# aosokin/os2d

Measured on AMD Instinct MI355X. Metric: query-image-pairs/s (1280-px input, ResNet50, N-class), higher is better.
Workload: dtype fftx3 (as fft; the per-bin complex GEMM on the fp16 MFMA with spectra split into fp16 hi+lo, 3 MFMAs per product, fp32 accumulate)

## Files before the change

### os2d_amd/csrc/dft_mfma.h

```cpp
#pragma once

#ifndef DFT_DEV
#error "the includer defines DFT_DEV, DFT_TID, DFT_BID, DFT_GRID, DFT_LDS, DFT_BARRIER, DFT_MFMA, DFT_SHFL_XOR, DFT_SHFL_XOR_U32, DFT_BALLOT, DFT_FLAG, DFT_FLAG_SET, DFT_RAISE, DFT_UNIFORM"
#endif

#ifndef DFT_HD
#define DFT_HD static inline
#endif
#ifndef DFT_MEMBER
#define DFT_MEMBER inline
#endif
#ifndef DFT_LANDED
#define DFT_LANDED(X)
#endif
#ifndef DFT_SWAP1
#define DFT_SWAP1(V) DFT_SHFL_XOR(V, 1)
#endif
#ifndef DFT_FWD_PREFETCH_AFTER
#define DFT_FWD_PREFETCH_AFTER 2
#endif
#ifndef DFT_INV_PREFETCH_AFTER
#define DFT_INV_PREFETCH_AFTER 2
#endif
#ifndef DFT_PIPE_REGA
#define DFT_PIPE_REGA 1
#endif
#ifndef DFT_PIPE_LDS
#define DFT_PIPE_LDS 1
#endif
#ifndef DFT_SCHED_FENCE
#define DFT_SCHED_FENCE()
#endif
#ifndef DFT_STREAM_STORE
#define DFT_STREAM_STORE(P, V) (*(P) = (V))
#endif
#ifndef DFT_STAMP
#define DFT_STAMP(K)
#define DFT_STAMP_BEGIN()
#define DFT_STAMP_END(BASE)
#endif

#include "tile_common.h"

namespace os2d_dft {

typedef float f32x4u __attribute__((ext_vector_type(4), aligned(4)));

constexpr int DFT_THR = 512, DFT_WAVES = 8;
constexpr int DFT_G = 4;
constexpr int DFT_MAXP = 64;
constexpr int DFT_MAXV = 48;
constexpr int DFT_MAXWK = 96;
constexpr int DFT_KREG = 8;
constexpr int DFT_OUT_SHB = 0, DFT_OUT_SHB_BORDERS = 1, DFT_OUT_PLANES = 2;

struct DftPlan {
  int H, W;
  int P, Q, V, NBINS;
  int T, TY, TX, TH, TW;
  int oy, ox;
  int LH, LW;
  int RH;
  int Pp;
  int Wk;
  int N1;
  int M2;
  int Mx;
  int N2;
  int MA;
  int MB;
  int KB;
  int NBo;
  int G;
  int eT;
  int fast;
  unsigned inv_cg, inv_t, inv_tx, inv_c4, inv_v, inv_pq, inv_og, inv_kg, inv_pp;
  int lds_const, lds_union, lds_total;
};

DFT_HD int dft_round_up(int x, int m) { return (x + m - 1) / m * m; }
DFT_HD unsigned dft_magic(unsigned d) { return d > 1 ? (unsigned)(((1ull << 32) + d - 1) / d) : 0u; }

DFT_HD int dft_units_fqt(int P, int Q) { return (dft_round_up(Q, 16) / 8) * 2 * dft_round_up(Q + 2, 32); }
constexpr int DFT_R2_P = 64, DFT_R2_MATU = 8 * 2 * 64, DFT_R2_TWU = 16;
constexpr int DFT_R2_LDS_TW = 512;
DFT_HD bool dft_radix2(int P) { return P == DFT_R2_P; }
DFT_HD int dft_units_fp2(int P, int Q) {
  return dft_radix2(P) ? DFT_R2_MATU + DFT_R2_TWU : (2 * dft_round_up(P, 8) / 8) * 2 * dft_round_up(2 * P, 32);
}
DFT_HD int dft_units_e2(int P, int Q) { return (2 * dft_round_up(P, 8) / 8) * 2 * dft_round_up(2 * P, 32); }
DFT_HD int dft_units_gq(int P, int Q) { return (dft_round_up(Q + 2, 16) / 8) * 2 * dft_round_up(Q, 32); }
DFT_HD size_t dft_matrices_units(int P, int Q) {
  return (size_t)dft_units_fqt(P, Q) + dft_units_fp2(P, Q) + dft_units_e2(P, Q) + dft_units_gq(P, Q);
}

static inline bool dft_plan_transform(int LH, int LW, int RH, int ncols, int minP, int minQ, int G, DftPlan* pl) {
  pl->G = G;
  pl->P = dft_round_up(minP, 4);
  if (pl->P == 60) pl->P = DFT_R2_P;
  pl->Q = dft_round_up(minQ, 2);
  pl->V = pl->Q / 2 + 1;
  pl->NBINS = dft_round_up(pl->P * pl->V, 8);
  pl->LH = LH;
  pl->LW = LW;
  pl->RH = RH;
  pl->Pp = dft_round_up(pl->P, 8);
  pl->Wk = dft_round_up(LW, 16);
  pl->N1 = dft_round_up(2 * pl->V, 32);
  pl->M2 = dft_round_up(2 * pl->P, 32);
  pl->Mx = dft_round_up(G * pl->Pp, 32);
  pl->N2 = dft_round_up(G * pl->V, 32);
  pl->MA = dft_round_up(2 * RH, 32);
  pl->MB = G * (pl->MA / 2);
  pl->KB = dft_round_up(2 * pl->V, 16);
  pl->NBo = dft_round_up(ncols, 32);
  int e = 0;
  while ((1 << e) < pl->P) ++e;
  pl->eT = e + 1;
  if (pl->P > DFT_MAXP || pl->V > DFT_MAXV || pl->Wk > DFT_MAXWK || LH > pl->P || LW > pl->Q || RH > pl->P) return false;
  const int fqt = (pl->Wk / 8) * 2 * pl->N1 * 16, gq = (pl->KB / 8) * 2 * pl->NBo * 16;
  const int x = (pl->Wk / 8) * 2 * (pl->Mx + 1) * 16, r2 = (2 * pl->Pp / 8) * 2 * (pl->N2 + 1) * 16;
  const int xs = pl->V * (pl->P * 8 * G + 16);
  const int y2 = r2, tt = (pl->KB / 8) * 2 * (pl->MB + 1) * 16;
  int u = x;
  if (r2 > u) u = r2;
  if (xs > u) u = xs;
  if (y2 > u) u = y2;
  if (tt > u) u = tt;
  if (G == 8) {
    if (dft_radix2(pl->P)) return false;
    const int fp2 = (2 * pl->Pp / 8) * 2 * pl->M2 * 16;
    const int ca = fqt + fp2, cb = gq + fp2;
    pl->lds_const = ca > cb ? ca : cb;
    pl->lds_union = dft_round_up(u, 256);
    pl->lds_total = pl->lds_const + pl->lds_union + 1024;
    const int t1 = (pl->Mx / 32) * (pl->N1 / 32), t2 = (pl->M2 / 32) * (pl->N2 / 32), tA = (pl->MA / 32) * (pl->N2 / 32),
              tB = (pl->MB / 32) * (pl->NBo / 32);
    const int npos = pl->Pp * (pl->Wk / 4), nitem = G * pl->V * (pl->Pp / 8);
    return pl->lds_total <= 160 * 1024 && t1 <= 24 && t2 <= 24 && tA <= 24 && tB <= 24 && npos <= 2 * DFT_THR && nitem <= 3 * DFT_THR;
  }
  pl->lds_const = fqt > gq ? fqt : gq;
  pl->lds_union = dft_round_up(u, 256);
  pl->lds_total = pl->lds_const + pl->lds_union + 1024;
  return pl->lds_total <= 160 * 1024;
}

static inline void dft_set_tiles(DftPlan* pl, int H, int W, int TY, int TX, int TH, int TW) {
  pl->H = H;
  pl->W = W;
  pl->TY = TY;
  pl->TX = TX;
  pl->T = TY * TX;
  pl->TH = TH;
  pl->TW = TW;
  pl->oy = TY > 1 ? 3 : 0;
  pl->ox = TX > 1 ? 3 : 0;
  pl->fast = (pl->T == 1 && (W & 3) == 0) ? 1 : 0;
  pl->inv_t = dft_magic((unsigned)pl->T);
  pl->inv_tx = dft_magic((unsigned)TX);
  pl->inv_c4 = dft_magic((unsigned)(pl->Wk / 4));
  pl->inv_v = dft_magic((unsigned)pl->V);
  pl->inv_pq = dft_magic((unsigned)(pl->P / 4 * pl->G * 2));
  pl->inv_kg = dft_magic((unsigned)(pl->Pp / 8));
  pl->inv_pp = dft_magic((unsigned)pl->Pp);
}

struct DftSize {
  int P, Q;
};
static const DftSize DFT_CANONICAL[6] = {{36, 46}, {44, 54}, {48, 62}, {52, 68}, {56, 70}, {64, 84}};

static inline bool dft_make_plan_policy(int H, int W, int canonical, DftPlan* out, int G = DFT_G) {
  bool found = false;
  long best = 0;
  for (int TY = 1; TY <= 48; ++TY)
    for (int TX = 1; TX <= 48; ++TX) {
      const int TH = (H + TY - 1) / TY, TW = (W + TX - 1) / TX;
      if ((TY > 1 && (TY - 1) * TH >= H) || (TX > 1 && (TX - 1) * TW >= W)) continue;
      const int LH = TY > 1 ? TH + 6 : H, LW = TX > 1 ? TW + 6 : W;
      const int minP = TY > 1 ? TH + 6 : H + 3, minQ = TX > 1 ? TW + 6 : W + 3;
      if (minP > DFT_MAXP || minQ > 2 * (DFT_MAXV - 1)) continue;
      for (int k = 0; k < (canonical ? 6 : 1); ++k) {
        if (canonical && (DFT_CANONICAL[k].P < minP || DFT_CANONICAL[k].Q < minQ)) continue;
        DftPlan c = {};
        if (!dft_plan_transform(LH, LW, TY > 1 ? TH + 3 : H, TX > 1 ? TW + 3 : W, canonical ? DFT_CANONICAL[k].P : minP,
                                canonical ? DFT_CANONICAL[k].Q : minQ, G, &c))
          continue;
        dft_set_tiles(&c, H, W, TY, TX, TH, TW);
        const long cost = (long)c.T * c.NBINS;
        if (!found || cost < best) {
          found = true;
          best = cost;
          *out = c;
        }
      }
    }
  return found;
}

#ifndef OS2D_HOST_EMU
static inline int dft_size_policy() {
  static const int policy = [] {
    const char* e = getenv("OS2D_DFT_SIZES");
    return (e && (e[0] == 'e' || e[0] == '0')) ? 0 : 1;
  }();
  return policy;
}
#else
static inline int dft_size_policy() { return emu_dft_policy; }
#endif
static inline bool dft_make_plan(int H, int W, DftPlan* out) { return dft_make_plan_policy(H, W, dft_size_policy(), out); }
static inline bool dft_plan_g8(const DftPlan& base, DftPlan* out) {
  DftPlan c = {};
  if (!dft_plan_transform(base.LH, base.LW, base.RH, base.TX > 1 ? base.TW + 3 : base.W, base.P, base.Q, 8, &c)) return false;
  dft_set_tiles(&c, base.H, base.W, base.TY, base.TX, base.TH, base.TW);
  *out = c;
  return true;
}

constexpr int DFT_PBLK = 64;
DFT_HD size_t dft_spectra_pair0(int pr, int NBT, int NQ, int cstride, size_t* qstride) {
  const int pb = pr / DFT_PBLK, pl = pr - pb * DFT_PBLK;
  const int nbl = NBT - pb * DFT_PBLK < DFT_PBLK ? NBT - pb * DFT_PBLK : DFT_PBLK;
  *qstride = (size_t)nbl * cstride * 8;
  return ((size_t)pb * DFT_PBLK * NQ + pl) * cstride * 8;
}

DFT_DEV int dft_div(int x, unsigned magic) { return magic ? (int)(((unsigned long long)(unsigned)x * magic) >> 32) : x; }

DFT_DEV void dft_split4(float a, float b, float c, float d, u32x2* hi, u32x2* lo) {
  const f32x4 x = {a, b, c, d};
  const half4 h = __builtin_convertvector(x, half4);
  *hi = __builtin_bit_cast(u32x2, h);
#ifdef DFT_SPLIT_LO_PAIR
  u32x2 l;
  l[0] = DFT_SPLIT_LO_PAIR(a, b, (*hi)[0]);
  l[1] = DFT_SPLIT_LO_PAIR(c, d, (*hi)[1]);
  *lo = l;
#else
  const half4 l = __builtin_convertvector(x - __builtin_convertvector(h, f32x4), half4);
  *lo = __builtin_bit_cast(u32x2, l);
#endif
}

DFT_DEV half8 dft_frag(const u32x4* p) { return __builtin_bit_cast(half8, *p); }

DFT_DEV f32x16 dft_mma3(half8 ah, half8 al, half8 bh, half8 bl, f32x16 acc) {
  acc = DFT_MFMA(ah, bl, acc);
  acc = DFT_MFMA(al, bh, acc);
  acc = DFT_MFMA(ah, bh, acc);
  return acc;
}

template <int NT, int KS>
DFT_DEV void dft_product_rega(f32x16* acc, const half8* ah, const half8* al, int ksn, const u32x4* B, int bstride, int nt0,
                              int ntstep, int l31, int hw) {
  constexpr int KR = KS ? KS : DFT_KREG;
  half8 bh[2][NT], bl[2][NT];
#define DFT_REGA_READ(KSTEP, SET)                                                                                          \
  _Pragma("unroll") for (int j = 0; j < NT; ++j) {                                                                         \
    bh[SET][j] = dft_frag(B + (size_t)((2 * (KSTEP) + hw) * 2 + 0) * bstride + (nt0 + ntstep * j) * 32 + l31);             \
    bl[SET][j] = dft_frag(B + (size_t)((2 * (KSTEP) + hw) * 2 + 1) * bstride + (nt0 + ntstep * j) * 32 + l31);             \
  }
  if (DFT_PIPE_REGA) DFT_REGA_READ(0, 0)
#pragma unroll
  for (int ks = 0; ks < KR; ++ks) {
    if (KS || ks < ksn) {
      if (DFT_PIPE_REGA) {
        if (ks + 1 < KR && (KS || ks + 1 < ksn)) DFT_REGA_READ(ks + 1, (ks + 1) & 1)
        DFT_SCHED_FENCE();
      } else {
        DFT_REGA_READ(ks, ks & 1)
      }
#pragma unroll
      for (int j = 0; j < NT; ++j) acc[j] = dft_mma3(ah[ks], al[ks], bh[ks & 1][j], bl[ks & 1][j], acc[j]);
      if (DFT_PIPE_REGA) DFT_SCHED_FENCE();
    }
  }
#undef DFT_REGA_READ
}

template <int KS>
DFT_DEV void dft_product_rega_any(f32x16* acc, int ntiles, const half8* ah, const half8* al, int ksn, const u32x4* B, int bstride,
                                  int nt0, int ntstep, int l31, int hw) {
  if (ntiles == 3) dft_product_rega<3, KS>(acc, ah, al, ksn, B, bstride, nt0, ntstep, l31, hw);
  else if (ntiles == 2) dft_product_rega<2, KS>(acc, ah, al, ksn, B, bstride, nt0, ntstep, l31, hw);
  else if (ntiles == 1) dft_product_rega<1, KS>(acc, ah, al, ksn, B, bstride, nt0, ntstep, l31, hw);
}

template <int NT, bool SHARE, int NW, int PIPE_MODE>
DFT_DEV void dft_product_lds(f32x16* acc, int ks0, int ks1, const u32x4* A, int astride, const u32x4* B, int bstride, int t0, int mtn,
                             int l31, int hw) {
  constexpr int NA = SHARE ? 1 : NT;
  int tm[NT], tn[NT];
#pragma unroll
  for (int j = 0; j < NT; ++j) {
    const int t = t0 + NW * j;
    tn[j] = t / mtn;
    tm[j] = t - tn[j] * mtn;
  }
  half8 ah[2][NA], al[2][NA], bh[2][NT], bl[2][NT];
#define DFT_LDS_READ(KSTEP, SET)                                                                                           \
  {                                                                                                                        \
    const int kc_ = (KSTEP) < ks1 ? (KSTEP) : ks1 - 1;                                                                     \
    _Pragma("unroll") for (int j = 0; j < NA; ++j) {                                                                       \
      ah[SET][j] = dft_frag(A + (size_t)((2 * kc_ + hw) * 2 + 0) * astride + tm[j] * 32 + l31);                            \
      al[SET][j] = dft_frag(A + (size_t)((2 * kc_ + hw) * 2 + 1) * astride + tm[j] * 32 + l31);                            \
    }                                                                                                                      \
    _Pragma("unroll") for (int j = 0; j < NT; ++j) {                                                                       \
      bh[SET][j] = dft_frag(B + (size_t)((2 * kc_ + hw) * 2 + 0) * bstride + tn[j] * 32 + l31);                            \
      bl[SET][j] = dft_frag(B + (size_t)((2 * kc_ + hw) * 2 + 1) * bstride + tn[j] * 32 + l31);                            \
    }                                                                                                                      \
  }
#define DFT_LDS_MMA(SET)                                                                                                   \
  DFT_SCHED_FENCE();                                                                                                       \
  _Pragma("unroll") for (int j = 0; j < NT; ++j)                                                                           \
    acc[j] = dft_mma3(ah[SET][SHARE ? 0 : j], al[SET][SHARE ? 0 : j], bh[SET][j], bl[SET][j], acc[j]);                    \
  DFT_SCHED_FENCE();
  if (ks0 >= ks1) return;
  constexpr bool PIPE = PIPE_MODE == 2 || (PIPE_MODE == 1 && SHARE);
  if (!PIPE) {
    for (int ks = ks0; ks < ks1; ++ks) {
      DFT_LDS_READ(ks, 0)
      _Pragma("unroll") for (int j = 0; j < NT; ++j)
        acc[j] = dft_mma3(ah[0][SHARE ? 0 : j], al[0][SHARE ? 0 : j], bh[0][j], bl[0][j], acc[j]);
    }
    return;
  }
  DFT_LDS_READ(ks0, 0)
  int ks = ks0;
  for (; ks + 1 < ks1; ks += 2) {
    DFT_LDS_READ(ks + 1, 1)
    DFT_LDS_MMA(0)
    DFT_LDS_READ(ks + 2, 0)
    DFT_LDS_MMA(1)
  }
  if (ks < ks1) {
    DFT_LDS_MMA(0)
  }
#undef DFT_LDS_READ
#undef DFT_LDS_MMA
}

template <int NW, int PIPE_MODE>
DFT_DEV void dft_product_lds_any(f32x16* acc, int ntiles, int ks0, int ks1, const u32x4* A, int astride, const u32x4* B, int bstride,
                                 int t0, int mtn, int l31, int hw) {
  const bool share = mtn == NW;
  if (ntiles == 3) {
    if (share) dft_product_lds<3, true, NW, PIPE_MODE>(acc, ks0, ks1, A, astride, B, bstride, t0, mtn, l31, hw);
    else dft_product_lds<3, false, NW, PIPE_MODE>(acc, ks0, ks1, A, astride, B, bstride, t0, mtn, l31, hw);
  } else if (ntiles == 2) {
    if (share) dft_product_lds<2, true, NW, PIPE_MODE>(acc, ks0, ks1, A, astride, B, bstride, t0, mtn, l31, hw);
    else dft_product_lds<2, false, NW, PIPE_MODE>(acc, ks0, ks1, A, astride, B, bstride, t0, mtn, l31, hw);
  } else if (ntiles == 1) {
    dft_product_lds<1, true, NW, PIPE_MODE>(acc, ks0, ks1, A, astride, B, bstride, t0, mtn, l31, hw);
  }
}

DFT_DEV void dft_matrix_unit(int which, int unit, int P, int Q, const double* twP, const double* twQ, u32x4* out) {
  const int V = Q / 2 + 1;
  const bool r2 = which == 1 && dft_radix2(P);
  if (r2 && unit >= DFT_R2_MATU) {
    const int u = 2 * (unit - DFT_R2_MATU);
    u32x4 o;
    for (int t = 0; t < 4; ++t) o[t] = __builtin_bit_cast(unsigned, (float)twP[2 * u + t]);
    *out = o;
    return;
  }
  const int tws = r2 ? 2 : 1;
  if (r2) P /= 2;
  const int Pp = dft_round_up(P, 8);
  int cols, kidx, hl, col;
  double vals[8];
  if (which == 0) cols = dft_round_up(2 * V, 32);
  else if (which == 1 || which == 2) cols = dft_round_up(2 * P, 32);
  else cols = dft_round_up(Q, 32);
  col = unit % cols;
  hl = (unit / cols) & 1;
  kidx = unit / (2 * cols);
  for (int t = 0; t < 8; ++t) {
    const int k = kidx * 8 + t;
    double x = 0.0;
    if (which == 0) {
      const int v = col >> 1, ri = col & 1;
      if (k < Q && v < V) x = twQ[2 * (int)(((long long)v * k) % Q) + ri] * 16384.0;
    } else if (r2) {
      const int h = 8 * (2 * (kidx >> 1) + (t >> 2)) + 4 * (kidx & 1) + (t & 3), u = col & 31;
      if (kidx < 4) {
        const int a = (int)(((long long)u * h) % P) * tws;
// ... 283 lines not shown
      for (int j = 0; j < 3; ++j) {
        const int t = wv + NW * j;
        const int nt = ALDS ? t / mt2n : (wv >> 2) + (NW / 4) * j;
        const bool mine = ALDS ? t < mt2n * nt2n : (nt < nt2n && mt2 < mt2n);
        un[j] = mine ? nt : -1;
        um[j] = ALDS ? t - nt * mt2n : mt2;
        nt2w += mine ? 1 : 0;
#pragma unroll
        for (int r = 0; r < 16; ++r) xc[j][r] = 0.f;
      }
      const int itn = it + DFT_GRID < iters ? it + DFT_GRID : it;
      {
        if (ALDS) {
          dft_product_lds_any<NW, DFT_PIPE_LDS ? 2 : 0>(xc, nt2w, 0, ks2n, ldsP, pl.M2, ldsU, N2S, wv, mt2n, l31, hw);
          DFT_FWD_PREFETCH_SLOTS(itn, tl, 0, NSLOT)
        } else if (DFT_FWD_PREFETCH_AFTER == 1 || (DFT_FWD_PREFETCH_AFTER == 2 && KS2 > 0 && KS2 <= 6)) {
          dft_product_rega_any<KS2>(xc, nt2w, fp2h, fp2l, ks2n, ldsU, N2S, wv >> 2, NW / 4, l31, hw);
          DFT_FWD_PREFETCH_SLOTS(itn, tl, 0, NSLOT)
        } else {
          DFT_FWD_PREFETCH_SLOTS(itn, tl, 0, NSLOT)
          dft_product_rega_any<KS2>(xc, nt2w, fp2h, fp2l, ks2n, ldsU, N2S, wv >> 2, NW / 4, l31, hw);
        }
      }
      DFT_BARRIER();
      DFT_STAMP(3)

      const int XS = P * 8 * G + 16;
#pragma unroll
      for (int j = 0; j < 3; ++j) {
        if (un[j] < 0) continue;
        const int n2 = un[j] * 32 + l31;
        const int img = dft_div(n2, pl.inv_v), v = n2 - img * V;
#pragma unroll
        for (int q = 0; q < 4; ++q) {
          const int u0 = (um[j] * 32 + 8 * q + 4 * hw) >> 1;
          if (img < G && u0 < P) {
            const float sc = 1.0f / 4194304.0f;
            f32x4 o;
            o[0] = xc[j][4 * q] * sc;
            o[1] = xc[j][4 * q + 1] * sc;
            o[2] = xc[j][4 * q + 2] * sc;
            o[3] = xc[j][4 * q + 3] * sc;
            *reinterpret_cast<f32x4*>(ldsUb + (size_t)v * XS + (u0 >> 2) * (G * 32) + img * 32 + (u0 & 3) * 8) = o;
          }
        }
      }
      DFT_BARRIER();
      DFT_STAMP(4)
    }

    {
      const int XS = P * 8 * G + 16;
      const int per_v = (P / 4) * (G * 2), npieces = V * per_v;
      size_t qstride;
      float* dstbase = X + dft_spectra_pair0(pr_, NBT, pl.NBINS / 4, Cpad, &qstride) + (size_t)c0_ * 8;
      if (R2) {
        constexpr int per_h = (DFT_R2_P / 8) * (G * 2);
        for (int i = tl; i < V * per_h; i += THR) {
          const int v = i / per_h, rem = i - v * per_h;
          const int uq = rem / (2 * G), jj = rem - uq * (2 * G);
          const unsigned char* src = ldsUb + (size_t)v * XS + uq * (G * 32) + jj * 16;
          const f32x4 e = *reinterpret_cast<const f32x4*>(src);
          const f32x4 o = *reinterpret_cast<const f32x4*>(src + (DFT_R2_P / 8) * (G * 32));
          const f32x4 w = *reinterpret_cast<const f32x4*>(ldsTw + (4 * uq + 2 * (jj & 1)) * 8);
          f32x4 t;
          t[0] = w[0] * o[0] - w[1] * o[1];
          t[1] = w[0] * o[1] + w[1] * o[0];
          t[2] = w[2] * o[2] - w[3] * o[3];
          t[3] = w[2] * o[3] + w[3] * o[2];
          float* dst = dstbase + (size_t)(v * (P / 4) + uq) * qstride + jj * 4;
          DFT_STREAM_STORE(reinterpret_cast<f32x4*>(dst), e + t);
          DFT_STREAM_STORE(reinterpret_cast<f32x4*>(dst + (size_t)(DFT_R2_P / 8) * qstride), e - t);
        }
      } else
      for (int i = tl; i < npieces; i += THR) {
        const int v = dft_div(i, pl.inv_pq), rem = i - v * per_v;
        const int uq = rem / (2 * G), jj = rem - uq * (2 * G);
        const f32x4 val = *reinterpret_cast<const f32x4*>(ldsUb + (size_t)v * XS + uq * (G * 32) + jj * 16);
        DFT_STREAM_STORE(reinterpret_cast<f32x4*>(dstbase + (size_t)(v * (P / 4) + uq) * qstride + jj * 4), val);
      }
      const int qpad0 = (P * V) / 4, qpad1 = pl.NBINS / 4;
      for (int i = tl; i < (qpad1 - qpad0) * 2 * G; i += THR)
        *reinterpret_cast<f32x4*>(dstbase + (size_t)(qpad0 + i / (2 * G)) * qstride + (i % (2 * G)) * 4) = f32x4{0.f, 0.f, 0.f, 0.f};
    }
    DFT_BARRIER();
    DFT_STAMP(5)
  }
  DFT_STAMP_END(0)
#undef DFT_FWD_ITER
#undef DFT_FWD_POS
#undef DFT_FWD_PREFETCH
#undef DFT_FWD_PREFETCH_SLOTS
}

template <bool TILED, int KSA = 0, int G = DFT_G>
DFT_DEV void dft_inverse_body(const float* Y,
                              const float* bp,
                              int MTP, unsigned char* out,
                              const u32x4* E2, const u32x4* Gq, const DftPlan& pl, int Cout, int NBT, int PLANE, int Ws,
                              int BASE, int iters, DFT_FLAG bad_flag, int zero_borders) {
  unsigned char* smem = DFT_LDS;
  const int tid = DFT_TID, lane = tid & 63, l31 = lane & 31, hw = lane >> 5;
  const int wv = DFT_UNIFORM(tid >> 6);
  const int P = pl.P, V = pl.V, Pp = pl.Pp, N2 = pl.N2, MB = pl.MB, KB = pl.KB, NBo = pl.NBo, H = pl.H, W = pl.W;
  const int N2S = N2 + 1, MBS = MB + 1;
  const int OG = Cout / G;
  constexpr bool ALDS = G == 8;
  constexpr int LG = G == 8 ? 3 : 2;
  u32x4* ldsG = reinterpret_cast<u32x4*>(smem);
  u32x4* ldsU = reinterpret_cast<u32x4*>(smem + pl.lds_const);
  unsigned char* ldsUb = smem + pl.lds_const;
  float* smaxw = reinterpret_cast<float*>(smem + pl.lds_const + pl.lds_union);
  const int nG = (KB / 8) * 2 * NBo, NQ = dft_round_up(pl.Q, 32);
  for (int i = tid; i < nG; i += DFT_THR) {
    const int kh = i / NBo, n = i - kh * NBo;
    ldsG[i] = Gq[(size_t)kh * NQ + n];
  }
  const int MAfull = dft_round_up(2 * P, 32);
  u32x4* ldsE = ldsG + nG;
  if (ALDS)
    for (int i = tid; i < (2 * Pp / 8) * 2 * MAfull; i += DFT_THR) ldsE[i] = E2[i];

  const int mtAn = pl.MA / 32, ntAn = N2 / 32, ksAn = 2 * Pp / 16;
  const int mtBn = MB / 32, ntBn = NBo / 32, ksBn = KB / 16;
  const int mtA = wv & 3;
  constexpr int KRA = KSA ? KSA : DFT_KREG;
  half8 e2h[KRA], e2l[KRA];
  if (!ALDS) {
#pragma unroll
    for (int ks = 0; ks < KRA; ++ks) {
      const int kc = ks < ksAn ? ks : 0, mc = mtA < mtAn ? mtA : 0;
      e2h[ks] = dft_frag(E2 + ((size_t)((2 * kc + hw) * 2 + 0)) * MAfull + mc * 32 + l31);
      e2l[ks] = dft_frag(E2 + ((size_t)((2 * kc + hw) * 2 + 1)) * MAfull + mc * 32 + l31);
    }
#pragma unroll
    for (int ks = 0; ks < KRA; ++ks) {
      DFT_LANDED(e2h[ks]);
      DFT_LANDED(e2l[ks]);
    }
  }

  constexpr int NITEM = 3;
  const int uoct = Pp / 8, nitem = G * V * uoct;
  f32x4 py[NITEM][4];
#define DFT_INV_PREFETCH(IT, TID) DFT_INV_PREFETCH_ITEMS(IT, TID, 0, NITEM)
#define DFT_INV_PREFETCH_ITEMS(IT, TID, S0, S1)                                             \
  {                                                                                         \
    const int pr_ = dft_div((IT), pl.inv_og), og_ = (IT)-pr_ * OG;                          \
    size_t qstride;                                                                         \
    const float* src_ = Y + dft_spectra_pair0(pr_, NBT, pl.NBINS / 4, Cout, &qstride) + (size_t)og_ * G * 8; \
    _Pragma("unroll") for (int s = (S0); s < (S1); ++s) {                                   \
      const int e_ = (TID) + s * DFT_THR;                                                   \
      const int ec_ = e_ < nitem ? e_ : 0;                                                  \
      const int pimg_ = ec_ & (G - 1), prest_ = ec_ >> LG;                                  \
      const int pv_ = dft_div(prest_, pl.inv_kg), puo_ = prest_ - pv_ * (Pp / 8);           \
      const int q0_ = pv_ * (P / 4) + 2 * puo_;                                             \
      const bool ptwo_ = 8 * puo_ + 4 < P;                                                  \
      const float* p0_ = src_ + (size_t)q0_ * qstride + pimg_ * 8;                          \
      const float* p1_ = src_ + (size_t)(ptwo_ ? q0_ + 1 : q0_) * qstride + pimg_ * 8;      \
      py[s][0] = *reinterpret_cast<const f32x4*>(p0_);                                     \
      py[s][1] = *reinterpret_cast<const f32x4*>(p0_ + 4);                                 \
      py[s][2] = *reinterpret_cast<const f32x4*>(p1_);                                     \
      py[s][3] = *reinterpret_cast<const f32x4*>(p1_ + 4);                                 \
    }                                                                                       \
  }
#define DFT_INV_ITEM(E)                                                                     \
  const int img_ = (E) & (G - 1), rest_ = (E) >> LG;                                        \
  const int v_ = dft_div(rest_, pl.inv_kg), uo_ = rest_ - v_ * uoct;                        \
  const bool two_ = 8 * uo_ + 4 < P;
#define DFT_INV_MAXIMA(TID)                                                                 \
  {                                                                                         \
    float m = 0.f;                                                                          \
    _Pragma("unroll") for (int s = 0; s < NITEM; ++s)                                       \
      if ((TID) + s * DFT_THR < nitem) {                                                    \
        DFT_INV_ITEM((TID) + s * DFT_THR)                                                   \
        (void)img_;                                                                         \
        (void)v_;                                                                           \
        (void)uo_;                                                                          \
        _Pragma("unroll") for (int k = 0; k < 4; ++k)                                       \
          if (k < 2 || two_) {                                                              \
            _Pragma("unroll") for (int e = 0; e < 4; ++e) m = fmaxf(m, fabsf(py[s][k][e])); \
          }                                                                                 \
      }                                                                                     \
    if (G == 4) m = fmaxf(m, DFT_SHFL_XOR(m, 4));                                           \
    m = fmaxf(m, DFT_SHFL_XOR(m, 8));                                                       \
    m = fmaxf(m, DFT_SHFL_XOR(m, 16));                                                      \
    m = fmaxf(m, DFT_SHFL_XOR(m, 32));                                                      \
    if (lane < G) smaxw[wv * G + lane] = m;                                                 \
  }
  bool bad = false;
  const int first = (DFT_GRID & 7) == 0 ? (DFT_BID & 7) * (DFT_GRID >> 3) + (DFT_BID >> 3) : DFT_BID;
  if (first < iters) {
    DFT_INV_PREFETCH(first, tid)
    DFT_INV_MAXIMA(tid)
  }
  DFT_BARRIER();

  DFT_STAMP_BEGIN()
  for (int it = first; it < iters; it += DFT_GRID) {
    int tl = tid;
#ifndef OS2D_HOST_EMU
    asm volatile("" : "+v"(tl));
#endif
    const int lane = tl & 63, l31 = lane & 31, hw = lane >> 5;
    const int pr = dft_div(it, pl.inv_og), og = it - pr * OG;
    const int nb = TILED ? dft_div(pr, pl.inv_t) : pr, tile = TILED ? pr - nb * pl.T : 0;
    const int ty = TILED ? dft_div(tile, pl.inv_tx) : 0, tx = TILED ? tile - ty * pl.TX : 0;
    const int y0 = TILED ? ty * pl.TH : 0, x0 = TILED ? tx * pl.TW : 0, oy = TILED ? pl.oy : 0, ox = TILED ? pl.ox : 0;
    const int TH_ = TILED ? pl.TH : H, TW_ = TILED ? pl.TW : W;
    const int o0 = og * G;

    DFT_STAMP(0)
    float simg = 1.f, cinv[4] = {0.f, 0.f, 0.f, 0.f};
    {
#pragma unroll
      for (int g = 0; g < G; ++g) {
        float m = 0.f;
#pragma unroll
        for (int w = 0; w < DFT_WAVES; ++w) m = fmaxf(m, smaxw[w * G + g]);
        int E = (int)((__builtin_bit_cast(unsigned, m) >> 23) & 0xffu) - 127;
        if (!(m > 0.f) || E < -100) E = -100;
        if (E > 100) E = 100;
        const float s = __builtin_bit_cast(float, (unsigned)(13 - E + 127) << 23);
        const float sinv = __builtin_bit_cast(float, (unsigned)(E - 13 + 127) << 23);
        if (g == (tl & (G - 1))) simg = s;
        const float ci = sinv * __builtin_bit_cast(float, (unsigned)(pl.eT - 13 + 127) << 23) / (float)(P * pl.Q);
        if (G == 4 || (g >> 2) == hw) cinv[g & 3] = ci;
      }
    }
#pragma unroll
    for (int s = 0; s < NITEM; ++s) {
      const int e = tl + s * DFT_THR;
      if (e < nitem) {
        DFT_INV_ITEM(e)
        const int img = img_, v = v_, uo = uo_;
        const bool two = two_;
        float re[8], im[8];
#pragma unroll
        for (int k = 0; k < 4; ++k) {
          const bool ok = k < 2 || two;
          re[2 * k] = ok ? py[s][k][0] * simg : 0.f;
          im[2 * k] = ok ? py[s][k][1] * simg : 0.f;
          re[2 * k + 1] = ok ? py[s][k][2] * simg : 0.f;
          im[2 * k + 1] = ok ? py[s][k][3] * simg : 0.f;
        }
        u32x2 h0, l0, h1, l1;
        u32x4 t;
        const size_t n = (size_t)img * V + v;
        dft_split4(re[0], re[1], re[2], re[3], &h0, &l0);
        dft_split4(re[4], re[5], re[6], re[7], &h1, &l1);
        t[0] = h0[0], t[1] = h0[1], t[2] = h1[0], t[3] = h1[1];
        ldsU[(size_t)((uo)*2 + 0) * N2S + n] = t;
        t[0] = l0[0], t[1] = l0[1], t[2] = l1[0], t[3] = l1[1];
        ldsU[(size_t)((uo)*2 + 1) * N2S + n] = t;
        dft_split4(im[0], im[1], im[2], im[3], &h0, &l0);
        dft_split4(im[4], im[5], im[6], im[7], &h1, &l1);
        t[0] = h0[0], t[1] = h0[1], t[2] = h1[0], t[3] = h1[1];
        ldsU[(size_t)((uoct + uo) * 2 + 0) * N2S + n] = t;
        t[0] = l0[0], t[1] = l0[1], t[2] = l1[0], t[3] = l1[1];
        ldsU[(size_t)((uoct + uo) * 2 + 1) * N2S + n] = t;
      }
    }
    DFT_BARRIER();
    DFT_STAMP(1)

    f32x16 ta[3];
    int an[3], am[3];
    int ntaw = 0;
#pragma unroll
    for (int j = 0; j < 3; ++j) {
      const int t = wv + DFT_WAVES * j;
      const int nt = ALDS ? t / mtAn : (wv >> 2) + 2 * j;
      const bool mine = ALDS ? t < mtAn * ntAn : (nt < ntAn && mtA < mtAn);
      an[j] = mine ? nt : -1;
      am[j] = ALDS ? t - nt * mtAn : mtA;
      ntaw += mine ? 1 : 0;
#pragma unroll
      for (int r = 0; r < 16; ++r) ta[j][r] = 0.f;
    }
    const int itn = it + DFT_GRID < iters ? it + DFT_GRID : it;
    {
      if (ALDS) {
        dft_product_lds_any<DFT_WAVES, DFT_PIPE_LDS ? 1 : 0>(ta, ntaw, 0, ksAn, ldsE, MAfull, ldsU, N2S, wv, mtAn, l31, hw);
        DFT_INV_PREFETCH_ITEMS(itn, tl, 0, NITEM)
      } else if (DFT_INV_PREFETCH_AFTER == 1 || (DFT_INV_PREFETCH_AFTER == 2 && KSA > 0 && KSA <= 6)) {
        dft_product_rega_any<KSA>(ta, ntaw, e2h, e2l, ksAn, ldsU, N2S, wv >> 2, 2, l31, hw);
        DFT_INV_PREFETCH_ITEMS(itn, tl, 0, NITEM)
      } else {
        DFT_INV_PREFETCH_ITEMS(itn, tl, 0, NITEM)
        dft_product_rega_any<KSA>(ta, ntaw, e2h, e2l, ksAn, ldsU, N2S, wv >> 2, 2, l31, hw);
      }
    }
    DFT_BARRIER();
    DFT_STAMP(2)

    {
      const float sc = __builtin_bit_cast(float, (unsigned)(127 - 14 - pl.eT) << 23);
#pragma unroll
      for (int j = 0; j < 3; ++j) {
        if (an[j] < 0) continue;
        const int n = an[j] * 32 + l31;
        const int img = dft_div(n, pl.inv_v), v = n - img * V;
        if (img >= G) continue;
#pragma unroll
        for (int q = 0; q < 4; ++q) {
          const int h0 = (am[j] * 32 + 8 * q + 4 * hw) >> 1;
          u32x2 hi, lo;
          dft_split4(ta[j][4 * q] * sc, ta[j][4 * q + 1] * sc, ta[j][4 * q + 2] * sc, ta[j][4 * q + 3] * sc, &hi, &lo);
          unsigned char* d0 = ldsUb + ((size_t)((v >> 2) * 2) * MBS + (size_t)h0 * G + img) * 16 + (v & 3) * 4;
          *reinterpret_cast<unsigned*>(d0) = hi[0];
          *reinterpret_cast<unsigned*>(d0 + (size_t)MBS * 16) = lo[0];
          *reinterpret_cast<unsigned*>(d0 + G * 16) = hi[1];
          *reinterpret_cast<unsigned*>(d0 + G * 16 + (size_t)MBS * 16) = lo[1];
        }
      }
      for (int v = V; v < KB / 2; ++v)
        for (int m = tl; m < MB; m += DFT_THR) {
          unsigned char* d0 = ldsUb + ((size_t)((v >> 2) * 2) * MBS + m) * 16 + (v & 3) * 4;
          *reinterpret_cast<unsigned*>(d0) = 0u;
          *reinterpret_cast<unsigned*>(d0 + (size_t)MBS * 16) = 0u;
        }
    }
    DFT_BARRIER();
    DFT_STAMP(3)

    f32x16 yc[3];
    int bm[3], bn[3];
    int ntbw = 0;
#pragma unroll
    for (int j = 0; j < 3; ++j) {
      const int t = wv + DFT_WAVES * j;
      const bool mine = t < mtBn * ntBn;
      bn[j] = mine ? t / mtBn : 0;
      bm[j] = mine ? t - bn[j] * mtBn : -1;
      ntbw += mine ? 1 : 0;
#pragma unroll
      for (int r = 0; r < 16; ++r) yc[j][r] = 0.f;
    }
    dft_product_lds_any<DFT_WAVES, DFT_PIPE_LDS ? 1 : 0>(yc, ntbw, 0, ksBn, ldsU, MBS, ldsG, NBo, wv, mtBn, l31, hw);
    DFT_INV_MAXIMA(tl)
    DFT_STAMP(4)

    {
      const bool planes = zero_borders == DFT_OUT_PLANES;
      float bias[4], osc[4];
#pragma unroll
      for (int g = 0; g < 4; ++g) {
        bias[g] = bp[o0 + (G == 8 ? 4 * hw : 0) + g];
        osc[g] = bp[2 * MTP + o0 + (G == 8 ? 4 * hw : 0) + g];
      }
      const int grp = o0 >> 3, slot = o0 & 7;
      unsigned char* hi_unit = out + (((size_t)nb * ((Cout + 7) >> 3) + grp) * 2 + 0) * (size_t)PLANE * 16 + slot * 2;
      unsigned char* lo_unit = out + (((size_t)nb * ((Cout + 7) >> 3) + grp) * 2 + 1) * (size_t)PLANE * 16 + slot * 2;
      if (zero_borders == DFT_OUT_SHB_BORDERS && (!TILED || tile == 0)) {
        const int rows = H * (Ws - W), tail0 = BASE + H * Ws, npad = BASE + rows + (PLANE - tail0);
        for (int k = tl; k < npad; k += DFT_THR) {
          int cell;
          if (k < BASE) cell = k;
          else if (k < BASE + rows) {
            const int jj = k - BASE, hr = jj / (Ws - W);
            cell = BASE + hr * Ws + W + (jj - hr * (Ws - W));
          } else cell = tail0 + (k - BASE - rows);
          if (G == 8) {
            *reinterpret_cast<u32x4*>(hi_unit + (size_t)cell * 16) = u32x4{0u, 0u, 0u, 0u};
            *reinterpret_cast<u32x4*>(lo_unit + (size_t)cell * 16) = u32x4{0u, 0u, 0u, 0u};
          } else {
            *reinterpret_cast<u32x2*>(hi_unit + (size_t)cell * 16) = u32x2{0u, 0u};
            *reinterpret_cast<u32x2*>(lo_unit + (size_t)cell * 16) = u32x2{0u, 0u};
          }
        }
      }
#pragma unroll
      for (int j = 0; j < 3; ++j) {
        if (bm[j] < 0) continue;
        const int wwin = bn[j] * 32 + l31, tw = wwin - ox;
#pragma unroll
        for (int q = 0; q < 4; ++q) {
          const int hwin = G == 8 ? bm[j] * 4 + q : (bm[j] * 32 + 8 * q + 4 * hw) >> 2, th = hwin - oy;
          const int h = y0 + th, w = x0 + tw;
          const bool inside = th >= 0 && th < TH_ && tw >= 0 && tw < TW_ && h < H && w < W;
          if (G == 8 || inside) {
            float t[4];
#pragma unroll
            for (int g = 0; g < 4; ++g) {
              const float pre = yc[j][4 * q + g] * cinv[g] + bias[g];
              t[g] = fmaxf(pre, 0.f) * osc[g];
              if (inside && (!(fabsf(t[g]) <= 65504.f) || pre != pre)) bad = true;
            }
            if (planes) {
              if (inside) {
                float* dst = reinterpret_cast<float*>(out) + ((size_t)nb * Cout + o0 + (G == 8 ? 4 * hw : 0)) * ((size_t)H * W) + (size_t)h * W + w;
#pragma unroll
                for (int g = 0; g < 4; ++g) dst[(size_t)g * H * W] = t[g] * (1.0f / 32768.0f);
              }
              continue;
            }
            u32x2 hi, lo;
            dft_split4(t[0], t[1], t[2], t[3], &hi, &lo);
            const size_t off = ((size_t)BASE + (size_t)h * Ws + w) * 16;
            if (G == 8) {
              const u32x2 send = hw ? hi : lo, keep = hw ? lo : hi;
              u32x2 recv;
              recv[0] = DFT_SHFL_XOR_U32(send[0], 32);
              recv[1] = DFT_SHFL_XOR_U32(send[1], 32);
              const u32x4 unit = hw ? u32x4{recv[0], recv[1], keep[0], keep[1]} : u32x4{keep[0], keep[1], recv[0], recv[1]};
              if (inside) *reinterpret_cast<u32x4*>((hw ? lo_unit : hi_unit) + off) = unit;
            } else {
              *reinterpret_cast<u32x2*>(hi_unit + off) = hi;
              *reinterpret_cast<u32x2*>(lo_unit + off) = lo;
            }
          }
        }
      }
    }
    DFT_BARRIER();
    DFT_STAMP(5)
  }
  DFT_STAMP_END(8)
  if (DFT_FLAG_SET(bad_flag) && DFT_BALLOT(bad) != 0ull) {
    if ((tid & 63) == 0) DFT_RAISE(bad_flag);
  }
#undef DFT_INV_MAXIMA
#undef DFT_INV_ITEM
#undef DFT_INV_PREFETCH
#undef DFT_INV_PREFETCH_ITEMS
}

}
```

### os2d_amd/csrc/spectral_f16.hip

```cpp
#include "tile_common.h"

namespace {


constexpr int SH_THR = 512;
constexpr int SH_WB = 4;
constexpr int SH_BINS = 8;
constexpr int SH_OH = 64, SH_NB = 64;
constexpr int SH_KC = 8;
constexpr int SH_STAGE = SH_WB * 2 * 2 * 64;
constexpr int SH_WSTAGE = 2 * SH_STAGE;
constexpr int SH_WRING = 2;

#define SH_MM(x_, y_, acc_) __builtin_amdgcn_mfma_f32_32x32x16_f16(x_, y_, acc_, 0, 0, 0)
__device__ __forceinline__ void sh_lds_barrier() { asm volatile("s_waitcnt lgkmcnt(0)\n\ts_barrier" ::: "memory"); }

template <bool XQ, bool R64>
__device__ __forceinline__ void spectral_gemm_f16_body(const u32x4* w16,
                                                       const float* __restrict__ wscale,
                                                       const f32x2* __restrict__ X,
                                                       f32x2* __restrict__ Y,
                                                       int NB, int C, int Cpad, int Cout, int NBINS, float xscale, int nunits) {
  extern __shared__ __attribute__((aligned(16))) unsigned char smem[];
  constexpr int JB = R64 ? SH_WB / 2 : SH_WB;
  constexpr int WSTAGE = R64 ? SH_STAGE : SH_WSTAGE;
  constexpr int NWL = WSTAGE / SH_THR, NXL = SH_STAGE / SH_THR;
  u32x4* ldsW = reinterpret_cast<u32x4*>(smem);
  u32x4* ldsX = ldsW + SH_WRING * WSTAGE;
  const int tid = threadIdx.x, lane = tid & 63, l31 = lane & 31, hw = lane >> 5;
  const int wv = __builtin_amdgcn_readfirstlane(tid >> 6);
  const int lidx = os2d_xcd_logical(blockIdx.x, gridDim.x);
  if (lidx >= nunits) return;
  constexpr int NBH = SH_BINS / SH_WB;
  const int bh = lidx % NBH, lg = lidx / NBH;
  const int nbt = (NB + SH_NB - 1) / SH_NB;
  const int bt = lg % nbt, g = lg / nbt;
  const int nb0 = bt * SH_NB, bin0 = g * SH_BINS + bh * SH_WB;
  const int KS = (C + SH_KC - 1) / SH_KC;
  const int ot = R64 ? wv & 1 : wv & 3, pt = R64 ? (wv >> 1) & 1 : wv >> 2;
  const int wbp = R64 ? wv >> 2 : 0;
  const int wq = wv & 3, wh = wv >> 2;

  f32x16 yr[JB], yi[JB];
#pragma unroll
  for (int j = 0; j < JB; ++j)
#pragma unroll
    for (int r = 0; r < 16; ++r) {
      yr[j][r] = 0.f;
      yi[j][r] = 0.f;
    }

  const u32x4* wbase = w16 + ((size_t)(g * 2 + (R64 ? 0 : wh)) * KS) * (SH_BINS * 256) + bh * SH_STAGE;
#define SH_WRUN(K) (R64 ? wv * 2 + (K) : wq * 4 + (K))
#define SH_WPART (R64 ? 0 : wh * SH_STAGE)
  u32x4 wra[NWL], wrb[NWL];
#define SH_LOAD_W(S, wr)                                                                                            \
  {                                                                                                                 \
    const u32x4* src_ = wbase + (size_t)(S) * (SH_BINS * 256);                                                      \
    _Pragma("unroll") for (int k_ = 0; k_ < NWL; ++k_) wr[k_] = src_[SH_WRUN(k_) * 64 + lane];                      \
  }
#define SH_LOAD_W1(S, wr, K) wr[K] = (wbase + (size_t)(S) * (SH_BINS * 256))[SH_WRUN(K) * 64 + lane];
#define SH_STORE_W(S, wr)                                                                                           \
  {                                                                                                                 \
    _Pragma("unroll") for (int k_ = 0; k_ < NWL; ++k_)                                                              \
        ldsW[((S) % SH_WRING) * WSTAGE + SH_WPART + SH_WRUN(k_) * 64 + lane] = wr[k_];                             \
  }
  const int xn = XQ ? wv * 8 + (lane >> 3) : wq * 16 + (lane & 15);
  const int xj = XQ ? (lane & 1) : (lane >> 4) & 1, xg = XQ ? (lane >> 2) & 1 : lane >> 5;
  const int xwh = XQ ? (lane >> 1) & 1 : wh;
  const bool xn_ok = nb0 + xn < NB;
  const int nbl = min(SH_NB, NB - nb0);
  const size_t qblk = XQ ? (size_t)nb0 * (NBINS >> 2) + (size_t)(bin0 >> 2) * nbl : 0;
  const f32x2* xrow = XQ ? X + ((qblk + min(xn, nbl - 1)) * Cpad) * 4 + 2 * xj
                         : X + (size_t)min(nb0 + xn, NB - 1) * NBINS + bin0 + 2 * xj;
  const size_t xcs = XQ ? 4 : (size_t)NB * NBINS;
  u32x4 pfa[2], pfb[2];
#define SH_LOAD_X(S, pfx)                                                                                           \
  {                                                                                                                 \
    _Pragma("unroll") for (int i_ = 0; i_ < 2; ++i_) {                                                              \
      const int c_ = min((S)*SH_KC + xg * 4 + xwh * 2 + i_, C - 1);                                                 \
      pfx[i_] = *reinterpret_cast<const u32x4*>(xrow + (size_t)c_ * xcs);                                           \
    }                                                                                                               \
  }
#define SH_LOAD_X1(S, pfx, I)                                                                                       \
  {                                                                                                                 \
    const int c_ = min((S)*SH_KC + xg * 4 + xwh * 2 + (I), C - 1);                                                  \
    pfx[I] = *reinterpret_cast<const u32x4*>(xrow + (size_t)c_ * xcs);                                              \
  }
#define SH_STORE_X(S, pfx)                                                                                          \
  {                                                                                                                 \
    _Pragma("unroll") for (int b2_ = 0; b2_ < 2; ++b2_) {                                                           \
      f32x4 v4_;                                                                                                    \
      _Pragma("unroll") for (int i_ = 0; i_ < 2; ++i_) {                                                            \
        const bool ok_ = xn_ok && (S)*SH_KC + xg * 4 + xwh * 2 + i_ < C;                                            \
        _Pragma("unroll") for (int p_ = 0; p_ < 2; ++p_) {                                                          \
          const unsigned raw_ = pfx[i_][2 * b2_ + p_];    \
          v4_[2 * i_ + p_] = ok_ ? __uint_as_float(raw_) * xscale : 0.f;                                            \
        }                                                                                                           \
      }                                                                                                             \
      const half4 h_ = __builtin_convertvector(v4_, half4);                                                         \
      const u32x2 hp_ = __builtin_bit_cast(u32x2, h_);      \
      const u32x2 lp_ = {os2d_split_lo_pair(v4_[0], v4_[1], hp_[0]), os2d_split_lo_pair(v4_[2], v4_[3], hp_[1])};    \
      const half4 l_ = __builtin_bit_cast(half4, lp_);                                                              \
      char* dst_ = reinterpret_cast<char*>(ldsX + ((S)&1) * SH_STAGE + (((2 * xj + b2_) * 2 + xg) * 2) * 64 + xn) + xwh * 8; \
      *reinterpret_cast<half4*>(dst_) = h_;                    \
      *reinterpret_cast<half4*>(dst_ + 64 * 16) = l_;                                                               \
    }                                                                                                               \
  }
#define SH_REQUEST1(SN, WN, PN, R)  \
  if constexpr ((R) < NWL) {                                                                                        \
    SH_LOAD_W1(SN, WN, R)                                                                                           \
  } else if constexpr ((R) < NWL + NXL) {                                                                           \
    SH_LOAD_X1(SN, PN, (R)-NWL)                                                                                     \
  }
#define SH_REQUEST2(SN, WN, PN, R)                                                                                  \
  if constexpr ((R) < NWL + NXL) {                                                                                  \
    SH_REQUEST1(SN, WN, PN, R)                                                                                      \
    SH_REQUEST1(SN, WN, PN, (R) + 1)                                                                                \
    __builtin_amdgcn_sched_barrier(0);                                                                              \
  }
#define SH_REQUESTS_HOOK(SN, WN, PN, J)                                                                             \
  if ((J) == 0) {                                                                                                   \
    SH_REQUEST2(SN, WN, PN, 0)                                                                                      \
  } else if ((J) == 1) {                                                                                            \
    SH_REQUEST2(SN, WN, PN, 2)                                                                                      \
  } else if ((J) == 2) {                                                                                            \
    SH_REQUEST2(SN, WN, PN, 4)                                                                                      \
  }
#define SH_COMPUTE(S, SN, WN, PN)                                                                                         \
  {                                                                                                                 \
                                         \
    const u32x4* aB = ldsW + ((S) % SH_WRING) * WSTAGE + (R64 ? wbp * JB * 256 : (ot >> 1) * SH_STAGE) +            \
                      (hw * 2) * 64 + (ot & 1) * 32 + l31;                                                          \
    const u32x4* bB = ldsX + ((S)&1) * SH_STAGE + wbp * JB * 256 + (hw * 2) * 64 + pt * 32 + l31;                   \
    half8 bq[2][2];                                                                                                 \
    u32x4 kq[2][2];                                                                                                 \
    bq[0][0] = *reinterpret_cast<const half8*>(bB);                                                                 \
    bq[0][1] = *reinterpret_cast<const half8*>(bB + 64);                                                            \
    kq[0][0] = aB[0];                                                                                               \
    kq[0][1] = aB[64];                                                                                              \
    _Pragma("unroll") for (int j = 0; j < JB; ++j) {                                                                \
      if (j + 1 < JB) {                                                                                             \
        bq[(j + 1) & 1][0] = *reinterpret_cast<const half8*>(bB + (j + 1) * 256);                                   \
        bq[(j + 1) & 1][1] = *reinterpret_cast<const half8*>(bB + (j + 1) * 256 + 64);                              \
        kq[(j + 1) & 1][0] = aB[(j + 1) * 256];                                                                     \
        kq[(j + 1) & 1][1] = aB[(j + 1) * 256 + 64];                                                                \
      }                                                                                                             \
      __builtin_amdgcn_sched_barrier(0);                                                                            \
      const half8 bhf = bq[j & 1][0], blf = bq[j & 1][1];                                                           \
      const u32x4 kh = kq[j & 1][0], kl = kq[j & 1][1];                       \
      u32x4 rh, rl, ih, il;                                                                                         \
      _Pragma("unroll") for (int d = 0; d < 4; ++d) {                                                               \
        rh[d] = kh[d] ^ 0x80000000u;                                                                 \
        rl[d] = kl[d] ^ 0x80000000u;                                                                                \
        ih[d] = __builtin_amdgcn_alignbit(kh[d], kh[d], 16);                                          \
        il[d] = __builtin_amdgcn_alignbit(kl[d], kl[d], 16);                                                        \
      }                                                                                                             \
      const half8 arh = __builtin_bit_cast(half8, rh), arl = __builtin_bit_cast(half8, rl);                         \
      const half8 aih = __builtin_bit_cast(half8, ih), ail = __builtin_bit_cast(half8, il);                         \
       \
      yr[j] = SH_MM(bhf, arl, yr[j]);                                                                               \
      yr[j] = SH_MM(blf, arh, yr[j]);                                                                               \
      yr[j] = SH_MM(bhf, arh, yr[j]);                                                                               \
      yi[j] = SH_MM(bhf, ail, yi[j]);                                                                               \
      yi[j] = SH_MM(blf, aih, yi[j]);                                                                               \
      yi[j] = SH_MM(bhf, aih, yi[j]);                                                                               \
      __builtin_amdgcn_sched_barrier(0);                                                                            \
      SH_REQUESTS_HOOK(SN, WN, PN, j)                                                                               \
    }                                                                                                               \
  }
#define SH_STEP(S, WC, PC, WN, PN)                                                                                  \
  {                                                                                                                 \
    const int sn_ = min((S) + 2, KS - 1);                                                                           \
    SH_COMPUTE(S, sn_, WN, PN)                                                                                      \
    __builtin_amdgcn_sched_barrier(0);                                                                              \
    SH_STORE_W((S) + 1, WC)                                                                                         \
    SH_STORE_X((S) + 1, PC)                                                                                         \
    sh_lds_barrier();                                                                                               \
  }
  SH_LOAD_W(0, wrb)
  SH_LOAD_X(0, pfb)
  SH_LOAD_W(min(1, KS - 1), wra)
  SH_LOAD_X(min(1, KS - 1), pfa)
  SH_STORE_W(0, wrb)
  SH_STORE_X(0, pfb)
  sh_lds_barrier();
  int s = 0;
  for (; s + 1 < KS; s += 2) {
    SH_STEP(s, wra, pfa, wrb, pfb)
    SH_STEP(s + 1, wrb, pfb, wra, pfa)
  }
  if (s < KS) SH_STEP(s, wra, pfa, wrb, pfb)
#undef SH_STEP
#undef SH_REQUESTS_HOOK
#undef SH_REQUEST1
#undef SH_REQUEST2
#undef SH_WRUN
#undef SH_WPART
#undef SH_LOAD_W1
#undef SH_LOAD_X1
#undef SH_LOAD_W
#undef SH_STORE_W
#undef SH_COMPUTE
#undef SH_LOAD_X
#undef SH_STORE_X

  const float inv_x = 1.0f / xscale;
  const int o = ot * 32 + l31;
  if (o < Cout) {
    const float sc = wscale[o] * inv_x;
#pragma unroll
    for (int r = 0; r < 16; ++r) {
      const int nb = nb0 + pt * 32 + (r & 3) + 8 * (r >> 2) + 4 * hw;
      if (nb < NB) {
        float4* dst = XQ ? reinterpret_cast<float4*>(Y + ((qblk + (nb - nb0)) * Cout + o) * 4)
                         : reinterpret_cast<float4*>(Y + (((size_t)(bin0 >> 2) * NB + nb) * Cout + o) * 4);
        if constexpr (R64) {
          dst[wbp] = make_float4(yr[0][r] * sc, yi[0][r] * sc, yr[1][r] * sc, yi[1][r] * sc);
        } else {
          dst[0] = make_float4(yr[0][r] * sc, yi[0][r] * sc, yr[1][r] * sc, yi[1][r] * sc);
          dst[1] = make_float4(yr[2][r] * sc, yi[2][r] * sc, yr[3][r] * sc, yi[3][r] * sc);
        }
      }
    }
  }
}

template <bool XQ>
__global__ __launch_bounds__(SH_THR, 1) void spectral_gemm_f16_kernel(const u32x4* w16, const float* __restrict__ wscale,
                                                                      const f32x2* __restrict__ X, f32x2* __restrict__ Y, int NB, int C,
                                                                      int Cpad, int Cout, int NBINS, int rows64, float xscale,
                                                                      int nunits) {
  if (rows64)
    spectral_gemm_f16_body<XQ, true>(w16, wscale, X, Y, NB, C, Cpad, Cout, NBINS, xscale, nunits);
  else
    spectral_gemm_f16_body<XQ, false>(w16, wscale, X, Y, NB, C, Cpad, Cout, NBINS, xscale, nunits);
}

}

size_t os2d_spectral_weight16_size(int C, int NBINS) {
  const size_t KS = (size_t)(C + SH_KC - 1) / SH_KC;
  return (size_t)(NBINS / SH_BINS) * 2 * KS * SH_BINS * 256 * 16 + 128 * sizeof(float);
}

float os2d_spectral_xscale_for(int H, int W) {
  float s = 1.0f;
  while (s * 2.0f * (float)H * (float)W <= 65504.0f) s *= 2.0f;
  return s;
}

int os2d_launch_spectral_gemm_f16(const void* w16, const float* X, float* Y, int NB, int C, int Cout, int NBINS, float xscale,
                                  int x_quads, int Cpad, hipStream_t stream) {
  if (NBINS % SH_BINS || Cout > 2 * SH_OH) {
    os2d_set_error("spectral_gemm_f16: NBINS %d must be a multiple of %d and Cout %d <= %d", NBINS, SH_BINS, Cout, 2 * SH_OH);
    return -3;
  }
  if (x_quads && Cpad < C) {
    os2d_set_error("spectral_gemm_f16: channel stride %d < C %d", Cpad, C);
    return -1;
  }
  static const bool rows64_env = [] {
    const char* e = getenv("OS2D_GEMM_ROWS64");
    return !(e && e[0] == '0');
  }();
  const bool r64 = Cout <= SH_OH && rows64_env;
  const int G = NBINS / SH_BINS, nbt = (NB + SH_NB - 1) / SH_NB;
  const size_t KS = (size_t)(C + SH_KC - 1) / SH_KC;
  const float* wscale = reinterpret_cast<const float*>(static_cast<const char*>(w16) + (size_t)G * 2 * KS * SH_BINS * 256 * 16);
  const size_t lds = (size_t)(SH_WRING * (r64 ? SH_STAGE : SH_WSTAGE) + 2 * SH_STAGE) * 16;
  const long long units = (long long)G * nbt * (SH_BINS / SH_WB);
  unsigned grid;
  if (int rc = os2d_xcd_grid(units, "spectral_gemm_f16", &grid)) return rc;
  auto kern = x_quads ? spectral_gemm_f16_kernel<true> : spectral_gemm_f16_kernel<false>;
  if (int rc = os2d_set_dynamic_lds(kern, lds, "spectral_gemm_f16")) return rc;
  hipLaunchKernelGGL(kern, dim3(grid), dim3(SH_THR), lds, stream, static_cast<const u32x4*>(w16), wscale,
                     reinterpret_cast<const f32x2*>(X), reinterpret_cast<f32x2*>(Y), NB, C, Cpad, Cout, NBINS, (int)r64, xscale, (int)units);
  return os2d_launched("spectral_gemm_f16");
}
```

Before: 48470.

## Simplify DFT epilogue addressing and pair spectral GEMM stores via LDS exchange

```diff
diff --git a/os2d_amd/csrc/dft_mfma.h b/os2d_amd/csrc/dft_mfma.h
--- a/os2d_amd/csrc/dft_mfma.h
+++ b/os2d_amd/csrc/dft_mfma.h
@@ -85,6 +85,9 @@
 constexpr int DFT_R2_P = 64, DFT_R2_MATU = 8 * 2 * 64, DFT_R2_TWU = 16;
 constexpr int DFT_R2_LDS_TW = 512;
 DFT_HD bool dft_radix2(int P) { return P == DFT_R2_P; }
+DFT_HD float dft_range_limit(float osc) {
+  return 65504.0f * __builtin_bit_cast(float, 0x7f000000u - __builtin_bit_cast(unsigned, osc));
+}
 DFT_HD int dft_units_fp2(int P, int Q) {
   return dft_radix2(P) ? DFT_R2_MATU + DFT_R2_TWU : (2 * dft_round_up(P, 8) / 8) * 2 * dft_round_up(2 * P, 32);
 }
@@ -974,24 +977,26 @@
         const int n = an[j] * 32 + l31;
         const int img = dft_div(n, pl.inv_v), v = n - img * V;
         if (img >= G) continue;
+        unsigned* dh = reinterpret_cast<unsigned*>(ldsUb) + ((unsigned)((v >> 2) * 2 * MBS + (am[j] * 16 + 2 * hw) * G + img) * 4u + (unsigned)(v & 3));
+        unsigned* dl = dh + (unsigned)MBS * 4u;
 #pragma unroll
         for (int q = 0; q < 4; ++q) {
-          const int h0 = (am[j] * 32 + 8 * q + 4 * hw) >> 1;
           u32x2 hi, lo;
           dft_split4(ta[j][4 * q] * sc, ta[j][4 * q + 1] * sc, ta[j][4 * q + 2] * sc, ta[j][4 * q + 3] * sc, &hi, &lo);
-          unsigned char* d0 = ldsUb + ((size_t)((v >> 2) * 2) * MBS + (size_t)h0 * G + img) * 16 + (v & 3) * 4;
-          *reinterpret_cast<unsigned*>(d0) = hi[0];
-          *reinterpret_cast<unsigned*>(d0 + (size_t)MBS * 16) = lo[0];
-          *reinterpret_cast<unsigned*>(d0 + G * 16) = hi[1];
-          *reinterpret_cast<unsigned*>(d0 + G * 16 + (size_t)MBS * 16) = lo[1];
-        }
-      }
-      for (int v = V; v < KB / 2; ++v)
-        for (int m = tl; m < MB; m += DFT_THR) {
-          unsigned char* d0 = ldsUb + ((size_t)((v >> 2) * 2) * MBS + m) * 16 + (v & 3) * 4;
-          *reinterpret_cast<unsigned*>(d0) = 0u;
-          *reinterpret_cast<unsigned*>(d0 + (size_t)MBS * 16) = 0u;
-        }
+          dh[q * (4 * G * 4)] = hi[0];
+          dh[q * (4 * G * 4) + G * 4] = hi[1];
+          dl[q * (4 * G * 4)] = lo[0];
+          dl[q * (4 * G * 4) + G * 4] = lo[1];
+        }
+      }
+      if (wv < KB / 2 - V) {
+        const int v = V + wv;
+        unsigned* d0 = reinterpret_cast<unsigned*>(ldsUb) + (unsigned)((v >> 2) * 2 * MBS) * 4u + (unsigned)(v & 3);
+        for (int m = lane; m < MB; m += 64) {
+          d0[(unsigned)m * 4u] = 0u;
+          d0[(unsigned)(m + MBS) * 4u] = 0u;
+        }
+      }
     }
     DFT_BARRIER();
     DFT_STAMP(3)
@@ -1015,11 +1020,13 @@
 
     {
       const bool planes = zero_borders == DFT_OUT_PLANES;
-      float bias[4], osc[4];
+      float bias[4], osc[4], lim[4];
 #pragma unroll
       for (int g = 0; g < 4; ++g) {
         bias[g] = bp[o0 + (G == 8 ? 4 * hw : 0) + g];
-        osc[g] = bp[2 * MTP + o0 + (G == 8 ? 4 * hw : 0) + g];
+        const float sc = bp[2 * MTP + o0 + (G == 8 ? 4 * hw : 0) + g];
+        lim[g] = dft_range_limit(sc);
+        osc[g] = planes ? sc * (1.0f / 32768.0f) : sc;
       }
       const int grp = o0 >> 3, slot = o0 & 7;
       unsigned char* hi_unit = out + (((size_t)nb * ((Cout + 7) >> 3) + grp) * 2 + 0) * (size_t)PLANE * 16 + slot * 2;
@@ -1042,34 +1049,40 @@
           }
         }
       }
+      const unsigned rows_in = (unsigned)(TH_ < H - y0 ? TH_ : H - y0), cols_in = (unsigned)(TW_ < W - x0 ? TW_ : W - x0);
+      const int hstep = G == 8 ? 1 : 2;
+      unsigned char* const plane0 = out + ((size_t)nb * Cout + o0) * ((size_t)H * W) * 4;
+      const unsigned HW4 = (unsigned)(H * W) * 4u;
 #pragma unroll
       for (int j = 0; j < 3; ++j) {
         if (bm[j] < 0) continue;
-        const int wwin = bn[j] * 32 + l31, tw = wwin - ox;
+        const int tw = bn[j] * 32 + l31 - ox;
+        const bool col_in = (unsigned)tw < cols_in;
+        const int th0 = (G == 8 ? bm[j] * 4 : bm[j] * 8 + hw) - oy;
+        const unsigned cell0 = planes ? (G == 8 ? 4u * hw * HW4 : 0u) + (unsigned)((y0 + th0) * W + x0 + tw) * 4u
+                                      : (unsigned)(BASE + (y0 + th0) * Ws + x0 + tw) * 16u;
+        const unsigned cstep = planes ? (unsigned)(hstep * W) * 4u : (unsigned)(hstep * Ws) * 16u;
 #pragma unroll
         for (int q = 0; q < 4; ++q) {
-          const int hwin = G == 8 ? bm[j] * 4 + q : (bm[j] * 32 + 8 * q + 4 * hw) >> 2, th = hwin - oy;
-          const int h = y0 + th, w = x0 + tw;
-          const bool inside = th >= 0 && th < TH_ && tw >= 0 && tw < TW_ && h < H && w < W;
+          const bool inside = col_in && (unsigned)(th0 + hstep * q) < rows_in;
           if (G == 8 || inside) {
             float t[4];
 #pragma unroll
             for (int g = 0; g < 4; ++g) {
               const float pre = yc[j][4 * q + g] * cinv[g] + bias[g];
               t[g] = fmaxf(pre, 0.f) * osc[g];
-              if (inside && (!(fabsf(t[g]) <= 65504.f) || pre != pre)) bad = true;
+              if (inside && !(pre <= lim[g])) bad = true;
             }
+            const unsigned off = cell0 + (unsigned)q * cstep;
             if (planes) {
               if (inside) {
-                float* dst = reinterpret_cast<float*>(out) + ((size_t)nb * Cout + o0 + (G == 8 ? 4 * hw : 0)) * ((size_t)H * W) + (size_t)h * W + w;
-#pragma unroll
-                for (int g = 0; g < 4; ++g) dst[(size_t)g * H * W] = t[g] * (1.0f / 32768.0f);
+#pragma unroll
+                for (int g = 0; g < 4; ++g) *reinterpret_cast<float*>(plane0 + (off + (unsigned)g * HW4)) = t[g];
               }
               continue;
             }
             u32x2 hi, lo;
             dft_split4(t[0], t[1], t[2], t[3], &hi, &lo);
-            const size_t off = ((size_t)BASE + (size_t)h * Ws + w) * 16;
             if (G == 8) {
               const u32x2 send = hw ? hi : lo, keep = hw ? lo : hi;
               u32x2 recv;
diff --git a/os2d_amd/csrc/spectral_f16.hip b/os2d_amd/csrc/spectral_f16.hip
--- a/os2d_amd/csrc/spectral_f16.hip
+++ b/os2d_amd/csrc/spectral_f16.hip
@@ -207,7 +207,44 @@
 
   const float inv_x = 1.0f / xscale;
   const int o = ot * 32 + l31;
-  if (o < Cout) {
+  if constexpr (R64) {
+    const float sc = o < Cout ? wscale[o] * inv_x : 0.f;
+    f32x4* xch = reinterpret_cast<f32x4*>(smem);
+#pragma unroll
+    for (int k = 0; k < 8; ++k) {
+      f32x4 t;
+      t[0] = (wbp ? yr[0][k] : yr[0][8 + k]) * sc;
+      t[1] = (wbp ? yi[0][k] : yi[0][8 + k]) * sc;
+      t[2] = (wbp ? yr[1][k] : yr[1][8 + k]) * sc;
+      t[3] = (wbp ? yi[1][k] : yi[1][8 + k]) * sc;
+      xch[(wv * 8 + k) * 64 + lane] = t;
+    }
+    sh_lds_barrier();
+    if (o < Cout) {
+#pragma unroll
+      for (int k = 0; k < 8; ++k) {
+        const int nb = nb0 + pt * 32 + (k & 3) + 8 * (k >> 2) + 4 * hw + 16 * wbp;
+        const f32x4 got = xch[((wv ^ 4) * 8 + k) * 64 + lane];
+        f32x4 own;
+        own[0] = (wbp ? yr[0][8 + k] : yr[0][k]) * sc;
+        own[1] = (wbp ? yi[0][8 + k] : yi[0][k]) * sc;
+        own[2] = (wbp ? yr[1][8 + k] : yr[1][k]) * sc;
+        own[3] = (wbp ? yi[1][8 + k] : yi[1][k]) * sc;
+        if (nb < NB) {
+          f32x4* dst = XQ ? reinterpret_cast<f32x4*>(Y + ((qblk + (nb - nb0)) * Cout + o) * 4)
+                          : reinterpret_cast<f32x4*>(Y + (((size_t)(bin0 >> 2) * NB + nb) * Cout + o) * 4);
+          f32x4 lo, hi;
+#pragma unroll
+          for (int e = 0; e < 4; ++e) {
+            lo[e] = wbp ? got[e] : own[e];
+            hi[e] = wbp ? own[e] : got[e];
+          }
+          dst[0] = lo;
+          dst[1] = hi;
+        }
+      }
+    }
+  } else if (o < Cout) {
     const float sc = wscale[o] * inv_x;
 #pragma unroll
     for (int r = 0; r < 16; ++r) {
@@ -215,12 +252,8 @@
       if (nb < NB) {
         float4* dst = XQ ? reinterpret_cast<float4*>(Y + ((qblk + (nb - nb0)) * Cout + o) * 4)
                          : reinterpret_cast<float4*>(Y + (((size_t)(bin0 >> 2) * NB + nb) * Cout + o) * 4);
-        if constexpr (R64) {
-          dst[wbp] = make_float4(yr[0][r] * sc, yi[0][r] * sc, yr[1][r] * sc, yi[1][r] * sc);
-        } else {
-          dst[0] = make_float4(yr[0][r] * sc, yi[0][r] * sc, yr[1][r] * sc, yi[1][r] * sc);
-          dst[1] = make_float4(yr[2][r] * sc, yi[2][r] * sc, yr[3][r] * sc, yi[3][r] * sc);
-        }
+        dst[0] = make_float4(yr[0][r] * sc, yi[0][r] * sc, yr[1][r] * sc, yi[1][r] * sc);
+        dst[1] = make_float4(yr[2][r] * sc, yi[2][r] * sc, yr[3][r] * sc, yi[3][r] * sc);
       }
     }
   }
```

New measurement: 48860, median of 6. Within noise of the previous version (+0.8%).
